# lean-dojo/ReProver

Measured on NVIDIA H100. Metric: premises encoded/sec (reindex_corpus, ByT5-small, seq_len<=512), higher is better.
Workload: dtype bf16

## Files before the change

### reprover_b200/csrc/rpx_encoder.cu

```cuda
#include <math.h>

#include <new>
#include <vector>

#include "rpx_gemm_launch.cuh"
#include "rpx_kernels.cuh"

namespace rpx {

namespace {

constexpr int kBlockN = 128;

int residual_gemm(const void* A, int64_t lda, const void* B, int64_t ldb, int T, int D, int K, float* h32,
                  __nv_bfloat16* h16, float* ss, cudaStream_t st) {
  EpiResidual::Params ep{h32, h16, D, ss, T};
  return launch_gemm<kBlockN, EpiResidual>(A, lda, B, ldb, T, D, K, ep, st);
}

struct LayerW {
  const __nv_bfloat16* qkv;
  const __nv_bfloat16* o;
  const __nv_bfloat16* wi;
  const __nv_bfloat16* wo;
};

struct ProfRec {
  int cls;
  cudaEvent_t a, b;
};

}

}

extern "C" int32_t rpx_t5_relative_bucket(int32_t relative_position, int32_t num_buckets, int32_t max_distance) {
  int nb = num_buckets / 2;
  int ret = relative_position > 0 ? nb : 0;
  int n = relative_position < 0 ? -relative_position : relative_position;
  const int max_exact = nb / 2;
  if (n < max_exact) return ret + n;
  float v = logf((float)n / (float)max_exact) / (float)log((double)max_distance / (double)max_exact) *
            (float)(nb - max_exact);
  int large = max_exact + (int)v;
  if (large > nb - 1) large = nb - 1;
  return ret + large;
}

struct rpx_encoder {
  rpx_t5_config cfg;
  int inner = 0;
  int n_parts = 0;
  int n_parts_lat = 0;
  int latency_tokens = 0;
  size_t layer_bytes = 0;
  const float* emb = nullptr;
  const float* final_ln = nullptr;
  const float* bias_lut = nullptr;
  std::vector<rpx::LayerW> layers;
  float* debug_hidden = nullptr;
  bool profiling = false;
  std::vector<rpx::ProfRec> prof_pending;
  std::vector<cudaEvent_t> event_pool;
  float prof_ms[RPX_N_KERNEL_CLASSES] = {0};
  int64_t prof_launches[RPX_N_KERNEL_CLASSES] = {0};
  std::vector<int32_t> h_cu_tokens;
  std::vector<int32_t> h_lens;
};

namespace rpx {

namespace {

struct PackedLayout {
  size_t emb, final_ln, bias_lut, bucket_tmp, layer0, layer_stride, qkv, o, wi, wo, total;
};

PackedLayout packed_layout(const rpx_t5_config& c) {
  PackedLayout L{};
  const size_t D = c.d_model, inner = (size_t)c.num_heads * c.d_kv, F = c.d_ff;
  size_t off = 0;
  auto take = [&](size_t bytes) {
    size_t o = off;
    off = align_up(off + bytes, 256);
    return o;
  };
  L.emb = take((size_t)c.vocab_size * D * 4);
  L.final_ln = take(D * 4);
  L.bias_lut = take((size_t)c.num_heads * (2 * c.rel_max_distance + 1) * 4);
  L.bucket_tmp = take((size_t)(2 * c.rel_max_distance + 1) * 4);
  L.layer0 = off;
  L.qkv = 0;
  size_t lo = 0;
  auto ltake = [&](size_t bytes) {
    size_t o = lo;
    lo = align_up(lo + bytes, 256);
    return o;
  };
  L.qkv = ltake(3 * inner * D * 2);
  L.o = ltake(D * inner * 2);
  L.wi = ltake(2 * F * D * 2);
// ... 109 lines not shown
  {
    Prof p(e, st, 1);
    EpiStoreBF16::Params ep{ws.qkv, 3 * inner, RowScale{ws.ssA, P, T, inv_d, c.ln_eps}};
    if (T <= kLatSmallMMaxTokens) {
      RPX_TRY((launch_gemm<kLatBlockN, EpiStoreBF16, false, kLatSmallStages, false, kLatSmallM>(ws.h16, D, w.qkv, D, T, 3 * inner,
                                                                                                 D, ep, st, 0, next_weights,
                                                                                                 next_bytes)));
    } else {
      RPX_TRY((launch_gemm<kLatBlockN, EpiStoreBF16, false, kLatStages>(ws.h16, D, w.qkv, D, T, 3 * inner, D, ep, st, 0,
                                                                         next_weights, next_bytes)));
    }
  }
  {
    Prof p(e, st, 2);
    RPX_TRY(launch_t5_attention(ws.qkv, ws.attn, ws.cu_tokens, e->bias_lut, T, S, max_len, c.num_heads, c.d_kv,
                                c.rel_max_distance, st));
  }
  {
    Prof p(e, st, 3);
    EpiResidual::Params ep{ws.h32, ws.h16, D, ws.ssB, T};
    if (T <= kLatSmallMMaxTokens) {
      RPX_TRY((launch_gemm<kLatBlockN, EpiResidualT<true>, false, kLatSmallStages, false, kLatSmallM>(ws.attn, inner, w.o, inner, T,
                                                                                                       D, inner, ep, st)));
    } else {
      RPX_TRY((launch_gemm<kLatBlockN, EpiResidualT<true>, false, kLatStages>(ws.attn, inner, w.o, inner, T, D, inner, ep, st)));
    }
  }
  {
    Prof p(e, st, 4);
    if (T <= kBlockM) {
      EpiGeGLUT<32>::Params ep{ws.ffn, F, RowScale{ws.ssB, P, T, inv_d, c.ln_eps}};
      RPX_TRY((launch_gemm<64, EpiGeGLUT<32>, false, kLatStages, true>(ws.h16, D, w.wi, D, T, 2 * F, D, ep, st)));
    } else {
      EpiGeGLUT<64>::Params ep{ws.ffn, F, RowScale{ws.ssB, P, T, inv_d, c.ln_eps}};
      RPX_TRY((launch_gemm<128, EpiGeGLUT<64>, false, kGemmStages, true>(ws.h16, D, w.wi, D, T, 2 * F, D, ep, st)));
    }
  }
  {
    Prof p(e, st, 5);
    EpiResidual::Params ep{ws.h32, ws.h16, D, ws.ssA, T};
    if (T <= kLatSmallMMaxTokens) {
      RPX_TRY((launch_gemm<kLatBlockN, EpiResidualT<true>, false, kLatSmallStages, false, kLatSmallM>(ws.ffn, F, w.wo, F, T, D, F,
                                                                                                       ep, st)));
    } else {
      RPX_TRY((launch_gemm<kLatBlockN, EpiResidualT<true>, false, kLatStages>(ws.ffn, F, w.wo, F, T, D, F, ep, st)));
    }
  }
  return RPX_OK;
}

int forward(rpx_encoder* e, const Workspace& ws, int T, int S, int max_len, void* d_out, int out_dtype,
            cudaStream_t st) {
  const rpx_t5_config& c = e->cfg;
  const int D = c.d_model, inner = e->inner, F = c.d_ff;
  const bool latency = T <= e->latency_tokens && D % 32 == 0 && (3 * inner) % 32 == 0;
  const int P = latency ? e->n_parts_lat : e->n_parts;
  const float inv_d = 1.0f / (float)D;
  struct PdlScope {
    explicit PdlScope(bool on) { set_pdl_scope(on); }
    ~PdlScope() { set_pdl_scope(false); }
  } pdl_scope(latency || T <= kPdlMaxTokens);
  {
    Prof p(e, st, 0);
    RPX_TRY(launch_embed(ws.ids, e->emb, ws.h32, ws.h16, ws.ssA, T, P, T, D, st));
  }
  auto dump = [&](int slab) -> int {
    if (e->debug_hidden)
      RPX_CUDA_OK(cudaMemcpyAsync(e->debug_hidden + (size_t)slab * T * D, ws.h32, (size_t)T * D * 4,
                                  cudaMemcpyDeviceToDevice, st));
    return RPX_OK;
  };
  RPX_TRY(dump(0));
  for (int l = 0; l < c.num_layers; ++l) {
    const LayerW& w = e->layers[l];
    if (latency) {
      const bool has_next = l + 1 < c.num_layers;
      RPX_TRY(forward_latency_layer(e, ws, w, has_next ? e->layers[l + 1].qkv : nullptr, has_next ? e->layer_bytes : 0, T, S,
                                    max_len, st));
      RPX_TRY(dump(l + 1));
      continue;
    }
    {
      Prof p(e, st, 1);
      EpiStoreBF16::Params ep{ws.qkv, 3 * inner, RowScale{ws.ssA, P, T, inv_d, c.ln_eps}};
      RPX_TRY((launch_gemm<kBlockN, EpiStoreBF16>(ws.h16, D, w.qkv, D, T, 3 * inner, D, ep, st)));
    }
    {
      Prof p(e, st, 2);
      RPX_TRY(launch_t5_attention(ws.qkv, ws.attn, ws.cu_tokens, e->bias_lut, T, S, max_len, c.num_heads, c.d_kv,
                                  c.rel_max_distance, st));
    }
    {
      Prof p(e, st, 3);
      RPX_TRY(residual_gemm(ws.attn, inner, w.o, inner, T, D, inner, ws.h32, ws.h16, ws.ssB, st));
    }
    {
      Prof p(e, st, 4);
      EpiWsGeGLU::Params ep{ws.ffn, F, RowScale{ws.ssB, P, T, inv_d, c.ln_eps}};
      RPX_TRY(launch_gemm_ws<EpiWsGeGLU>(ws.h16, D, w.wi, D, T, 2 * F, D, ep, st));
    }
    {
      Prof p(e, st, 5);
      RPX_TRY(residual_gemm(ws.ffn, F, w.wo, F, T, D, F, ws.h32, ws.h16, ws.ssA, st));
    }
    RPX_TRY(dump(l + 1));
  }
  {
    Prof p(e, st, 6);
    float* scratch = latency && (size_t)F * 2 >= (size_t)D * 4 ? reinterpret_cast<float*>(ws.ffn) : nullptr;
    RPX_TRY(launch_pool_normalize(ws.h32, ws.ssA, T, P, e->final_ln, ws.cu_tokens, d_out, out_dtype, S, D,
                                  c.ln_eps, st, scratch, max_len));
  }
  return RPX_OK;
}

}
}

using namespace rpx;

extern "C" {

size_t rpx_encoder_packed_bytes(const rpx_t5_config* cfg) {
  if (validate_cfg(cfg) != RPX_OK) return 0;
  return packed_layout(*cfg).total;
}

int rpx_encoder_create(const rpx_t5_config* cfg, const rpx_t5_weights* w, void* d_packed, size_t packed_bytes,
                       void* stream, rpx_encoder** out) {
  RPX_TRY(validate_cfg(cfg));
  RPX_REQUIRE(w && d_packed && out, RPX_ERR_INVALID, "rpx_encoder_create: null argument");
  DeviceInfo dev;
  RPX_TRY(get_device_info(&dev));
  const PackedLayout L = packed_layout(*cfg);
  RPX_REQUIRE(packed_bytes >= L.total, RPX_ERR_WORKSPACE, "packed buffer too small: %zu < %zu", packed_bytes, L.total);
  RPX_REQUIRE((reinterpret_cast<uintptr_t>(d_packed) & 255) == 0, RPX_ERR_INVALID, "packed buffer must be 256-byte aligned");
  cudaStream_t st = static_cast<cudaStream_t>(stream);
  uint8_t* base = static_cast<uint8_t*>(d_packed);
  const int D = cfg->d_model, inner = cfg->num_heads * cfg->d_kv, F = cfg->d_ff;

  rpx_encoder* e = new (std::nothrow) rpx_encoder();
  RPX_REQUIRE(e != nullptr, RPX_ERR_INVALID, "out of host memory");
  e->cfg = *cfg;
  e->inner = inner;
  e->n_parts = ceil_div(D, kBlockN) * (EpiResidual::kWarps / 4);
  e->n_parts_lat = ceil_div(D, 32) * (EpiResidual::kWarps / 4);
  auto fail = [&](int code) {
    delete e;
    return code;
  };
#define TRY_E(expr)                        \
  do {                                     \
    int _s = (expr);                       \
    if (_s != RPX_OK) return fail(_s);     \
  } while (0)
#define CUDA_E(expr)                                                                                   \
  do {                                                                                                 \
    cudaError_t _c = (expr);                                                                           \
    if (_c != cudaSuccess) {                                                                           \
      set_error("%s:%d: %s failed: %s", __FILE__, __LINE__, #expr, cudaGetErrorString(_c));           \
      return fail(RPX_ERR_CUDA);                                                                       \
    }                                                                                                  \
  } while (0)

  CUDA_E(cudaMemcpyAsync(base + L.emb, w->d_shared, (size_t)cfg->vocab_size * D * 4, cudaMemcpyDeviceToDevice, st));
  CUDA_E(cudaMemcpyAsync(base + L.final_ln, w->d_final_ln, (size_t)D * 4, cudaMemcpyDeviceToDevice, st));
  e->emb = reinterpret_cast<const float*>(base + L.emb);
  e->final_ln = reinterpret_cast<const float*>(base + L.final_ln);

  const int R = cfg->rel_max_distance, width = 2 * R + 1;
  std::vector<int32_t> buckets(width);
  for (int j = 0; j < width; ++j) buckets[j] = rpx_t5_relative_bucket(j - R, cfg->rel_buckets, R);
  CUDA_E(cudaMemcpyAsync(base + L.bucket_tmp, buckets.data(), (size_t)width * 4, cudaMemcpyHostToDevice, st));
  bias_lut_kernel<<<ceil_div(cfg->num_heads * width, 256), 256, 0, st>>>(
      w->d_rel_bias, reinterpret_cast<const int32_t*>(base + L.bucket_tmp), reinterpret_cast<float*>(base + L.bias_lut),
      cfg->num_heads, width);
  CUDA_E(cudaGetLastError());
  e->bias_lut = reinterpret_cast<const float*>(base + L.bias_lut);

  e->layers.resize(cfg->num_layers);
  for (int l = 0; l < cfg->num_layers; ++l) {
    uint8_t* lb = base + L.layer0 + L.layer_stride * l;
    __nv_bfloat16* qkv = reinterpret_cast<__nv_bfloat16*>(lb + L.qkv);
    __nv_bfloat16* o = reinterpret_cast<__nv_bfloat16*>(lb + L.o);
    __nv_bfloat16* wi = reinterpret_cast<__nv_bfloat16*>(lb + L.wi);
    __nv_bfloat16* wo = reinterpret_cast<__nv_bfloat16*>(lb + L.wo);
    TRY_E(launch_pack_weight(w->h_q[l], w->h_ln0[l], qkv, inner, D, 0, inner, inner, st));
    TRY_E(launch_pack_weight(w->h_k[l], w->h_ln0[l], qkv, inner, D, inner, inner, inner, st));
    TRY_E(launch_pack_weight(w->h_v[l], w->h_ln0[l], qkv, inner, D, 2 * inner, inner, inner, st));
    TRY_E(launch_pack_weight(w->h_o[l], nullptr, o, D, inner, 0, D, D, st));
    TRY_E(launch_pack_weight(w->h_wi0[l], w->h_ln1[l], wi, F, D, 0, 128, 256, st));
    TRY_E(launch_pack_weight(w->h_wi1[l], w->h_ln1[l], wi, F, D, 128, 128, 256, st));
    TRY_E(launch_pack_weight(w->h_wo[l], nullptr, wo, D, F, 0, D, D, st));
    e->layers[l] = LayerW{qkv, o, wi, wo};
    e->layer_bytes = L.layer_stride;
  }
  CUDA_E(cudaStreamSynchronize(st));
#undef TRY_E
#undef CUDA_E
  *out = e;
  return RPX_OK;
}

int rpx_encoder_destroy(rpx_encoder* enc) {
  if (!enc) return RPX_OK;
  for (auto& r : enc->prof_pending) {
    cudaEventDestroy(r.a);
    cudaEventDestroy(r.b);
  }
  for (auto ev : enc->event_pool) cudaEventDestroy(ev);
  delete enc;
  return RPX_OK;
}

size_t rpx_encoder_workspace_bytes(const rpx_encoder* enc, int64_t max_tokens, int64_t max_seqs) {
  if (!enc || max_tokens <= 0 || max_seqs <= 0) return 0;
  return carve(enc, nullptr, max_tokens, max_seqs).total;
}

int rpx_encode_bytes(rpx_encoder* enc, const uint8_t* d_bytes, const int64_t* h_offsets, int32_t n_seqs,
                     int32_t max_seq_len, void* d_out, int32_t out_dtype, void* d_workspace,
                     size_t workspace_bytes, void* stream) {
  RPX_REQUIRE(enc && h_offsets && d_out && d_workspace, RPX_ERR_INVALID, "rpx_encode_bytes: null argument");
  RPX_REQUIRE(n_seqs > 0, RPX_ERR_INVALID, "rpx_encode_bytes: n_seqs=%d", n_seqs);
  RPX_REQUIRE(max_seq_len >= 1, RPX_ERR_INVALID, "rpx_encode_bytes: max_seq_len=%d", max_seq_len);
  RPX_REQUIRE(h_offsets[0] >= 0, RPX_ERR_INVALID, "rpx_encode_bytes: negative offset");
  cudaStream_t st = static_cast<cudaStream_t>(stream);
  auto& cu = enc->h_cu_tokens;
// ... 108 lines not shown
```

### reprover_b200/csrc/rpx_gemm_api.cu

```cuda
#include "rpx_gemm_launch.cuh"

extern "C" int rpx_gemm_bf16_f32(const void* d_A, const void* d_B, float* d_C, int32_t M, int32_t N,
                                 int32_t K, void* stream) {
  using namespace rpx;
  RPX_REQUIRE(d_A && d_B && d_C, RPX_ERR_INVALID, "rpx_gemm_bf16_f32: null pointer");
  EpiWsStoreF32::Params ep{d_C, N};
  return launch_gemm_ws<EpiWsStoreF32>(d_A, K, d_B, K, M, N, K, ep, static_cast<cudaStream_t>(stream));
}

extern "C" int rpx_gemm2_bf16_f32(const void* d_A, const void* d_B, float* d_C, int32_t M, int32_t N, int32_t K,
                                  void* stream) {
  using namespace rpx;
  RPX_REQUIRE(d_A && d_B && d_C, RPX_ERR_INVALID, "rpx_gemm2_bf16_f32: null pointer");
  EpiStoreF32::Params ep{d_C, N};
  return launch_gemm_pair<EpiStoreF32>(d_A, K, d_B, K, M, N, K, ep, static_cast<cudaStream_t>(stream));
}
```

### reprover_b200/csrc/rpx_gemm_launch.cuh

```cuda
#pragma once
#include "rpx_common.cuh"
#include "rpx_gemm.cuh"
#include "rpx_gemm_ws.cuh"

namespace rpx {

constexpr int kGemmStages = 4;

template <int BLOCK_N, class Epi, bool M_FASTEST = false, int STAGES = kGemmStages, bool SPLIT_B = false, int BM = kBlockM>
int launch_gemm(const void* A, int64_t lda, const void* B, int64_t ldb, int M, int N, int K,
                const typename Epi::Params& ep, cudaStream_t stream, int grid_limit = 0, const void* prefetch_ptr = nullptr,
                size_t prefetch_bytes = 0) {
  using Cfg = GemmCfg<BLOCK_N, STAGES, BM>;
  static_assert(BM == kBlockM || (!M_FASTEST && Epi::kWarps == 4), "64-row tiles: encoder epilogues with one warp per lane group");
  RPX_REQUIRE(M > 0 && N > 0 && K > 0, RPX_ERR_INVALID, "gemm: empty problem M=%d N=%d K=%d", M, N, K);
  RPX_REQUIRE(K % kBlockK == 0, RPX_ERR_UNSUPPORTED, "gemm: K=%d must be a multiple of %d", K, kBlockK);
  RPX_REQUIRE(M_FASTEST || N % 32 == 0, RPX_ERR_UNSUPPORTED, "gemm: N=%d must be a multiple of 32", N);
  DeviceInfo dev;
  RPX_TRY(get_device_info(&dev));
  CUtensorMap tmA, tmB;
  RPX_TRY(make_tmap_bf16_2d(&tmA, A, (uint64_t)M, (uint64_t)K, (uint64_t)lda, BM));
  RPX_TRY(make_tmap_bf16_2d(&tmB, B, (uint64_t)N, (uint64_t)K, (uint64_t)ldb, SPLIT_B ? BLOCK_N / 2 : BLOCK_N));
  RPX_REQUIRE(!SPLIT_B || N % BLOCK_N == 0, RPX_ERR_UNSUPPORTED, "gemm: split-B tiles need N %% %d == 0", BLOCK_N);
  const int tiles_m = ceil_div(M, BM);
  const int tiles_n = ceil_div(N, BLOCK_N);
  const size_t smem = Cfg::smem_bytes(Epi::kSmemBytes);
  RPX_REQUIRE(smem <= dev.smem_optin, RPX_ERR_UNSUPPORTED, "gemm: needs %zu B smem, device allows %zu",
              smem, dev.smem_optin);
  auto kern = gemm_tc_kernel<BLOCK_N, STAGES, Epi, M_FASTEST, SPLIT_B, BM>;
  static thread_local int configured_dev = -1;
  if (configured_dev != dev.device) {
    RPX_CUDA_OK(cudaFuncSetAttribute(kern, cudaFuncAttributeMaxDynamicSharedMemorySize, (int)smem));
    configured_dev = dev.device;
  }
  int grid = tiles_m * tiles_n;
  int cap = grid_limit > 0 ? grid_limit : dev.num_sms;
  if (grid > cap) grid = cap;
  L2Prefetch pf{prefetch_ptr, (uint32_t)prefetch_bytes, grid, next_timeline_slot()};
  if (prefetch_ptr != nullptr && prefetch_bytes > 0 && prefetch_bytes < ((size_t)1 << 32) && grid < dev.num_sms)
    grid = dev.num_sms;
  RPX_CUDA_OK(launch_pdl(kern, dim3(grid), dim3(gemm_threads<Epi>()), smem, stream, pdl_enabled(), tmA, tmB, M, N, K, tiles_m,
                         tiles_n, 1, ep, pf));
  return RPX_OK;
}

template <class Epi>
int launch_gemm_ws(const void* A, int64_t lda, const void* B, int64_t ldb, int M, int N, int K,
                   const typename Epi::Params& ep, cudaStream_t stream) {
  RPX_REQUIRE(M > 0 && N > 0 && K > 0, RPX_ERR_INVALID, "gemm: empty problem M=%d N=%d K=%d", M, N, K);
  RPX_REQUIRE(K % kBlockK == 0, RPX_ERR_UNSUPPORTED, "gemm: K=%d must be a multiple of %d", K, kBlockK);
  RPX_REQUIRE(N % 32 == 0, RPX_ERR_UNSUPPORTED, "gemm: N=%d must be a multiple of 32", N);
  DeviceInfo dev;
  RPX_TRY(get_device_info(&dev));
  CUtensorMap tmA, tmB;
  RPX_TRY(make_tmap_bf16_2d(&tmA, A, (uint64_t)M, (uint64_t)K, (uint64_t)lda, kBlockM));
  RPX_TRY(make_tmap_bf16_2d(&tmB, B, (uint64_t)N, (uint64_t)K, (uint64_t)ldb, kWsBlockN));
  const int tiles_m = ceil_div(M, kBlockM);
  const int tiles_n = ceil_div(N, kWsBlockN);
  const size_t smem = WsCfg::kSmemBytes;
  RPX_REQUIRE(smem <= dev.smem_optin, RPX_ERR_UNSUPPORTED, "gemm: needs %zu B smem, device allows %zu", smem,
              dev.smem_optin);
  auto kern = gemm_ws_kernel<Epi>;
  static thread_local int configured_dev = -1;
  if (configured_dev != dev.device) {
    RPX_CUDA_OK(cudaFuncSetAttribute(kern, cudaFuncAttributeMaxDynamicSharedMemorySize, (int)smem));
    configured_dev = dev.device;
  }
  int grid = tiles_m * tiles_n;
  if (grid > dev.num_sms) grid = dev.num_sms;
  RPX_CUDA_OK(launch_pdl(kern, dim3(grid), dim3(kWsThreads), smem, stream, pdl_enabled(), tmA, tmB, M, N, K, tiles_m,
                         tiles_n, ep));
  return RPX_OK;
}

template <class Epi, int STAGES = kGemmStages>
int launch_gemm_pair(const void* A, int64_t lda, const void* B, int64_t ldb, int M, int N, int K,
                     const typename Epi::Params& ep, cudaStream_t stream) {
  constexpr int BLOCK_N = 128;
  using Cfg = GemmCfg<BLOCK_N, STAGES, kBlockM>;
  RPX_REQUIRE(M > 0 && N > 0 && K > 0, RPX_ERR_INVALID, "gemm: empty problem M=%d N=%d K=%d", M, N, K);
  RPX_REQUIRE(K % kBlockK == 0, RPX_ERR_UNSUPPORTED, "gemm: K=%d must be a multiple of %d", K, kBlockK);
  RPX_REQUIRE(N % 32 == 0, RPX_ERR_UNSUPPORTED, "gemm: N=%d must be a multiple of 32", N);
  DeviceInfo dev;
  RPX_TRY(get_device_info(&dev));
  CUtensorMap tmA, tmB;
  RPX_TRY(make_tmap_bf16_2d(&tmA, A, (uint64_t)M, (uint64_t)K, (uint64_t)lda, kBlockM));
  RPX_TRY(make_tmap_bf16_2d(&tmB, B, (uint64_t)N, (uint64_t)K, (uint64_t)ldb, BLOCK_N / 2));
  const int tiles_m = ceil_div(M, kBlockM);
  const int tiles_n = ceil_div(N, BLOCK_N);
  const size_t smem = Cfg::smem_bytes(Epi::kSmemBytes);
  RPX_REQUIRE(smem <= dev.smem_optin, RPX_ERR_UNSUPPORTED, "gemm: needs %zu B smem, device allows %zu", smem,
              dev.smem_optin);
  auto kern = gemm_tc_kernel<BLOCK_N, STAGES, Epi, false, false, kBlockM, true>;
  static thread_local int configured_dev = -1;
  if (configured_dev != dev.device) {
    RPX_CUDA_OK(cudaFuncSetAttribute(kern, cudaFuncAttributeMaxDynamicSharedMemorySize, (int)smem));
    configured_dev = dev.device;
  }
  int pairs = ceil_div(tiles_m, 2) * tiles_n;
  if (pairs > dev.num_sms / 2) pairs = dev.num_sms / 2;
  cudaLaunchConfig_t cfg{};
  cfg.gridDim = dim3(2 * pairs);
  cfg.blockDim = dim3(gemm_threads<Epi>());
  cfg.dynamicSmemBytes = smem;
  cfg.stream = stream;
  cudaLaunchAttribute at[1];
  at[0].id = cudaLaunchAttributeClusterDimension;
  at[0].val.clusterDim.x = 2;
  at[0].val.clusterDim.y = 1;
  at[0].val.clusterDim.z = 1;
  cfg.attrs = at;
  cfg.numAttrs = 1;
  RPX_CUDA_OK(cudaLaunchKernelEx(&cfg, kern, tmA, tmB, M, N, K, tiles_m, tiles_n, 1, ep,
                                 L2Prefetch{nullptr, 0u, 2 * pairs, next_timeline_slot()}));
  return RPX_OK;
}

}
```

### reprover_b200/csrc/rpx_gemm_ws.cuh

```cuda
#pragma once
#include "rpx_gemm.cuh"

namespace rpx {

constexpr int kWsBlockN = 256;
constexpr int kWsStages = 4;
constexpr int kWsThreads = 384;

struct WsCfg {
  static constexpr int kABytes = kBlockM * kBlockK * 2;
  static constexpr int kBBytes = kWsBlockN * kBlockK * 2;
  static constexpr int kStageBytes = kABytes + kBBytes;
  static constexpr size_t kSmemBytes = (size_t)kWsStages * kStageBytes + 1024 + 256;
};

struct FragCtx {
  int m0, n0;
  int n_blk;
  int n_cols;
  int M, N;
  int r0;
  int q;
};

template <class Epi>
__global__ void __launch_bounds__(kWsThreads, 1)
gemm_ws_kernel(const __grid_constant__ CUtensorMap tmA, const __grid_constant__ CUtensorMap tmB, int M, int N, int K,
               int tiles_m, int tiles_n, typename Epi::Params ep) {
  extern __shared__ uint8_t smem_raw[];
  const uint32_t raw_addr = smem_u32(smem_raw);
  uint8_t* smem = smem_raw + ((1024 - (raw_addr & 1023)) & 1023);
  uint8_t* sA = smem;
  uint8_t* sB = smem + kWsStages * WsCfg::kABytes;
  uint64_t* full = reinterpret_cast<uint64_t*>(smem + kWsStages * WsCfg::kStageBytes);
  uint64_t* empty = full + kWsStages;

  const int warp = threadIdx.x >> 5;
  const int wg = warp >> 2;
  const int num_kb = K / kBlockK;
  const int num_tiles = tiles_m * tiles_n;

  if (threadIdx.x == 0) {
    tma_prefetch_desc(&tmA);
    tma_prefetch_desc(&tmB);
    for (int s = 0; s < kWsStages; ++s) {
      mbar_init(&full[s], 1);
      mbar_init(&empty[s], 2 * 128);
    }
    fence_mbar_init();
  }
  __syncthreads();
  pdl_launch_dependents();
  pdl_wait();

  if (wg == 0) {
    setmaxnreg_dec<40>();
    if (warp == 0 && elect_one()) {
      int stage = 0;
      uint32_t phase = 0;
      for (int t = blockIdx.x; t < num_tiles; t += gridDim.x) {
        const int m_blk = t / tiles_n, n_blk = t % tiles_n;
        for (int kb = 0; kb < num_kb; ++kb) {
          mbar_wait(&empty[stage], phase ^ 1);
          mbar_arrive_expect_tx(&full[stage], WsCfg::kStageBytes);
          tma_load_2d(sA + stage * WsCfg::kABytes, &tmA, &full[stage], kb * kBlockK, m_blk * kBlockM);
          tma_load_2d(sB + stage * WsCfg::kBBytes, &tmB, &full[stage], kb * kBlockK, n_blk * kWsBlockN);
          if (++stage == kWsStages) {
            stage = 0;
            phase ^= 1;
          }
        }
      }
    }
  } else {
    setmaxnreg_inc<232>();
    const int cw = wg - 1;
    const int lane = threadIdx.x & 31;
    Epi epi(ep);
    float acc[128];
    int stage = 0;
    uint32_t phase = 0;
    for (int t = blockIdx.x; t < num_tiles; t += gridDim.x) {
      FragCtx c;
      c.n_blk = t % tiles_n;
      c.m0 = (t / tiles_n) * kBlockM;
      c.n0 = c.n_blk * kWsBlockN;
      c.n_cols = N - c.n0 < kWsBlockN ? N - c.n0 : kWsBlockN;
      c.M = M;
      c.N = N;
      c.r0 = c.m0 + 64 * cw + 16 * (warp & 3) + (lane >> 2);
      c.q = lane & 3;
      int prev = 0;
      for (int kb = 0; kb < num_kb; ++kb) {
        mbar_wait(&full[stage], phase);
        const uint64_t a_desc = make_smem_desc_kmajor_sw128(smem_u32(sA + stage * WsCfg::kABytes)) + 512 * cw;
        const uint64_t b_desc = make_smem_desc_kmajor_sw128(smem_u32(sB + stage * WsCfg::kBBytes));
        wgmma_fence_operand(acc);
        wgmma_fence();
#pragma unroll
        for (int k = 0; k < kBlockK / kMmaK; ++k) wgmma_m64n256k16_ss(acc, a_desc + 2 * k, b_desc + 2 * k, (kb | k) != 0);
        wgmma_commit();
        if (kb == 0) epi.prefetch(c);
        if (kb > 0) {
          wgmma_wait<1>();
          mbar_arrive(&empty[prev]);
        }
        prev = stage;
        if (++stage == kWsStages) {
          stage = 0;
          phase ^= 1;
        }
      }
      wgmma_wait<0>();
      wgmma_fence_operand(acc);
      mbar_arrive(&empty[prev]);
      epi.tile(c, acc);
    }
  }
}


struct EpiWsStoreF32 {
  using Params = EpiStoreF32::Params;
  Params p;
  __device__ explicit EpiWsStoreF32(const Params& p_) : p(p_) {}
  __device__ void prefetch(const FragCtx&) {}
  __device__ void tile(const FragCtx& c, const float (&acc)[128]) {
#pragma unroll
    for (int j = 0; j < 32; ++j) {
      if (8 * j < c.n_cols) {
        float* dst = p.C + (size_t)c.r0 * p.ldc + c.n0 + 8 * j + 2 * c.q;
        if (c.r0 < c.M) *reinterpret_cast<float2*>(dst) = make_float2(acc[4 * j], acc[4 * j + 1]);
        if (c.r0 + 8 < c.M) *reinterpret_cast<float2*>(dst + 8 * (size_t)p.ldc) = make_float2(acc[4 * j + 2], acc[4 * j + 3]);
      }
    }
  }
};

struct EpiWsGeGLU {
  struct Params {
    __nv_bfloat16* out;
    int ldo;
    RowScale rs;
  };
  Params p;
  float rs0 = 0.f, rs1 = 0.f;
  __device__ explicit EpiWsGeGLU(const Params& p_) : p(p_) {}
  __device__ void prefetch(const FragCtx& c) {
    rs0 = c.r0 < c.M ? p.rs.get(c.r0) : 0.f;
    rs1 = c.r0 + 8 < c.M ? p.rs.get(c.r0 + 8) : 0.f;
  }
  __device__ void tile(const FragCtx& c, const float (&acc)[128]) {
    __nv_bfloat16* dst = p.out + (size_t)c.r0 * p.ldo + c.n_blk * (kWsBlockN / 2) + 2 * c.q;
#pragma unroll
    for (int j = 0; j < 16; ++j) {
      const float* g = acc + 4 * j;
      const float* u = acc + 4 * (j + 16);
      if (c.r0 < c.M)
        *reinterpret_cast<uint32_t*>(dst + 8 * j) =
            pack_bf16x2(gelu_new(g[0] * rs0) * (u[0] * rs0), gelu_new(g[1] * rs0) * (u[1] * rs0));
      if (c.r0 + 8 < c.M)
        *reinterpret_cast<uint32_t*>(dst + 8 * (size_t)p.ldo + 8 * j) =
            pack_bf16x2(gelu_new(g[2] * rs1) * (u[2] * rs1), gelu_new(g[3] * rs1) * (u[3] * rs1));
    }
  }
};

}
```

### reprover_b200/csrc/rpx_ptx.cuh

```cuda
#pragma once
#include <cuda_runtime.h>
#include <cuda_bf16.h>
#include <stdint.h>

namespace rpx {

#define RPX_DEVICE __device__ __forceinline__

RPX_DEVICE uint32_t smem_u32(const void* p) {
  return static_cast<uint32_t>(__cvta_generic_to_shared(p));
}

RPX_DEVICE uint32_t lane_id() { return threadIdx.x & 31; }

RPX_DEVICE uint32_t elect_one() {
  uint32_t pred = 0;
  asm volatile(
      "{\n"
      ".reg .b32 rx;\n"
      ".reg .pred px;\n"
      "elect.sync rx|px, 0xFFFFFFFF;\n"
      "@px mov.s32 %0, 1;\n"
      "}\n"
      : "+r"(pred));
// ... 123 lines not shown
      "{\n"
      ".reg .b32 ra;\n"
      "mapa.shared::cluster.u32 ra, %0, %1;\n"
      "mbarrier.arrive.release.cluster.shared::cluster.b64 _, [ra];\n"
      "}\n" ::"r"(smem_u32(bar)),
      "r"(cta)
      : "memory");
}

RPX_DEVICE void wgmma_fence() { asm volatile("wgmma.fence.sync.aligned;" ::: "memory"); }
RPX_DEVICE void wgmma_commit() { asm volatile("wgmma.commit_group.sync.aligned;" ::: "memory"); }
template <int N>
RPX_DEVICE void wgmma_wait() {
  asm volatile("wgmma.wait_group.sync.aligned %0;" ::"n"(N) : "memory");
}
template <int R>
RPX_DEVICE void wgmma_fence_operand(float (&d)[R]) {
#pragma unroll
  for (int i = 0; i < R; ++i) asm volatile("" : "+f"(d[i])::"memory");
}

RPX_DEVICE void wgmma_m64n64k16_ss(float (&d)[32], uint64_t desc_a, uint64_t desc_b, uint32_t accumulate) {
  asm volatile(
      "{\n"
      ".reg .pred p;\n"
      "setp.ne.b32 p, %34, 0;\n"
      "wgmma.mma_async.sync.aligned.m64n64k16.f32.bf16.bf16 "
      "{%0, %1, %2, %3, %4, %5, %6, %7, %8, %9, %10, %11, %12, %13, %14, %15, %16, %17, %18, %19, %20, %21, %22, %23, %24, %25, %26, %27, %28, %29, %30, %31}, %32, %33, p, 1, 1, 0, 0;\n"
      "}\n"
      : "+f"(d[0]), "+f"(d[1]), "+f"(d[2]), "+f"(d[3]), "+f"(d[4]), "+f"(d[5]), "+f"(d[6]), "+f"(d[7]), "+f"(d[8]), "+f"(d[9]), "+f"(d[10]), "+f"(d[11]), "+f"(d[12]), "+f"(d[13]), "+f"(d[14]), "+f"(d[15]), "+f"(d[16]), "+f"(d[17]), "+f"(d[18]), "+f"(d[19]), "+f"(d[20]), "+f"(d[21]), "+f"(d[22]), "+f"(d[23]), "+f"(d[24]), "+f"(d[25]), "+f"(d[26]), "+f"(d[27]), "+f"(d[28]), "+f"(d[29]), "+f"(d[30]), "+f"(d[31])
      : "l"(desc_a), "l"(desc_b), "r"(accumulate));
}

RPX_DEVICE void wgmma_m64n128k16_ss(float (&d)[64], uint64_t desc_a, uint64_t desc_b, uint32_t accumulate) {
  asm volatile(
      "{\n"
      ".reg .pred p;\n"
      "setp.ne.b32 p, %66, 0;\n"
      "wgmma.mma_async.sync.aligned.m64n128k16.f32.bf16.bf16 "
      "{%0, %1, %2, %3, %4, %5, %6, %7, %8, %9, %10, %11, %12, %13, %14, %15, %16, %17, %18, %19, %20, %21, %22, %23, %24, %25, %26, %27, %28, %29, %30, %31, %32, %33, %34, %35, %36, %37, %38, %39, %40, %41, %42, %43, %44, %45, %46, %47, %48, %49, %50, %51, %52, %53, %54, %55, %56, %57, %58, %59, %60, %61, %62, %63}, %64, %65, p, 1, 1, 0, 0;\n"
      "}\n"
      : "+f"(d[0]), "+f"(d[1]), "+f"(d[2]), "+f"(d[3]), "+f"(d[4]), "+f"(d[5]), "+f"(d[6]), "+f"(d[7]), "+f"(d[8]), "+f"(d[9]), "+f"(d[10]), "+f"(d[11]), "+f"(d[12]), "+f"(d[13]), "+f"(d[14]), "+f"(d[15]), "+f"(d[16]), "+f"(d[17]), "+f"(d[18]), "+f"(d[19]), "+f"(d[20]), "+f"(d[21]), "+f"(d[22]), "+f"(d[23]), "+f"(d[24]), "+f"(d[25]), "+f"(d[26]), "+f"(d[27]), "+f"(d[28]), "+f"(d[29]), "+f"(d[30]), "+f"(d[31]), "+f"(d[32]), "+f"(d[33]), "+f"(d[34]), "+f"(d[35]), "+f"(d[36]), "+f"(d[37]), "+f"(d[38]), "+f"(d[39]), "+f"(d[40]), "+f"(d[41]), "+f"(d[42]), "+f"(d[43]), "+f"(d[44]), "+f"(d[45]), "+f"(d[46]), "+f"(d[47]), "+f"(d[48]), "+f"(d[49]), "+f"(d[50]), "+f"(d[51]), "+f"(d[52]), "+f"(d[53]), "+f"(d[54]), "+f"(d[55]), "+f"(d[56]), "+f"(d[57]), "+f"(d[58]), "+f"(d[59]), "+f"(d[60]), "+f"(d[61]), "+f"(d[62]), "+f"(d[63])
      : "l"(desc_a), "l"(desc_b), "r"(accumulate));
}

RPX_DEVICE void wgmma_m64n256k16_ss(float (&d)[128], uint64_t desc_a, uint64_t desc_b, uint32_t accumulate) {
  asm volatile(
      "{\n"
      ".reg .pred p;\n"
      "setp.ne.b32 p, %130, 0;\n"
      "wgmma.mma_async.sync.aligned.m64n256k16.f32.bf16.bf16 "
      "{%0, %1, %2, %3, %4, %5, %6, %7, %8, %9, %10, %11, %12, %13, %14, %15, %16, %17, %18, %19, %20, %21, %22, %23, %24, %25, %26, %27, %28, %29, %30, %31, %32, %33, %34, %35, %36, %37, %38, %39, %40, %41, %42, %43, %44, %45, %46, %47, %48, %49, %50, %51, %52, %53, %54, %55, %56, %57, %58, %59, %60, %61, %62, %63, %64, %65, %66, %67, %68, %69, %70, %71, %72, %73, %74, %75, %76, %77, %78, %79, %80, %81, %82, %83, %84, %85, %86, %87, %88, %89, %90, %91, %92, %93, %94, %95, %96, %97, %98, %99, %100, %101, %102, %103, %104, %105, %106, %107, %108, %109, %110, %111, %112, %113, %114, %115, %116, %117, %118, %119, %120, %121, %122, %123, %124, %125, %126, %127}, %128, %129, p, 1, 1, 0, 0;\n"
      "}\n"
      : "+f"(d[0]), "+f"(d[1]), "+f"(d[2]), "+f"(d[3]), "+f"(d[4]), "+f"(d[5]), "+f"(d[6]), "+f"(d[7]), "+f"(d[8]), "+f"(d[9]), "+f"(d[10]), "+f"(d[11]), "+f"(d[12]), "+f"(d[13]), "+f"(d[14]), "+f"(d[15]), "+f"(d[16]), "+f"(d[17]), "+f"(d[18]), "+f"(d[19]), "+f"(d[20]), "+f"(d[21]), "+f"(d[22]), "+f"(d[23]), "+f"(d[24]), "+f"(d[25]), "+f"(d[26]), "+f"(d[27]), "+f"(d[28]), "+f"(d[29]), "+f"(d[30]), "+f"(d[31]), "+f"(d[32]), "+f"(d[33]), "+f"(d[34]), "+f"(d[35]), "+f"(d[36]), "+f"(d[37]), "+f"(d[38]), "+f"(d[39]), "+f"(d[40]), "+f"(d[41]), "+f"(d[42]), "+f"(d[43]), "+f"(d[44]), "+f"(d[45]), "+f"(d[46]), "+f"(d[47]), "+f"(d[48]), "+f"(d[49]), "+f"(d[50]), "+f"(d[51]), "+f"(d[52]), "+f"(d[53]), "+f"(d[54]), "+f"(d[55]), "+f"(d[56]), "+f"(d[57]), "+f"(d[58]), "+f"(d[59]), "+f"(d[60]), "+f"(d[61]), "+f"(d[62]), "+f"(d[63]), "+f"(d[64]), "+f"(d[65]), "+f"(d[66]), "+f"(d[67]), "+f"(d[68]), "+f"(d[69]), "+f"(d[70]), "+f"(d[71]), "+f"(d[72]), "+f"(d[73]), "+f"(d[74]), "+f"(d[75]), "+f"(d[76]), "+f"(d[77]), "+f"(d[78]), "+f"(d[79]), "+f"(d[80]), "+f"(d[81]), "+f"(d[82]), "+f"(d[83]), "+f"(d[84]), "+f"(d[85]), "+f"(d[86]), "+f"(d[87]), "+f"(d[88]), "+f"(d[89]), "+f"(d[90]), "+f"(d[91]), "+f"(d[92]), "+f"(d[93]), "+f"(d[94]), "+f"(d[95]), "+f"(d[96]), "+f"(d[97]), "+f"(d[98]), "+f"(d[99]), "+f"(d[100]), "+f"(d[101]), "+f"(d[102]), "+f"(d[103]), "+f"(d[104]), "+f"(d[105]), "+f"(d[106]), "+f"(d[107]), "+f"(d[108]), "+f"(d[109]), "+f"(d[110]), "+f"(d[111]), "+f"(d[112]), "+f"(d[113]), "+f"(d[114]), "+f"(d[115]), "+f"(d[116]), "+f"(d[117]), "+f"(d[118]), "+f"(d[119]), "+f"(d[120]), "+f"(d[121]), "+f"(d[122]), "+f"(d[123]), "+f"(d[124]), "+f"(d[125]), "+f"(d[126]), "+f"(d[127])
      : "l"(desc_a), "l"(desc_b), "r"(accumulate));
}

RPX_DEVICE void wgmma_m64n64k16_rs_bmn(float (&d)[32], const uint32_t (&a)[4], uint64_t desc_b, uint32_t accumulate) {
  asm volatile(
      "{\n"
      ".reg .pred p;\n"
      "setp.ne.b32 p, %37, 0;\n"
      "wgmma.mma_async.sync.aligned.m64n64k16.f32.bf16.bf16 "
      "{%0, %1, %2, %3, %4, %5, %6, %7, %8, %9, %10, %11, %12, %13, %14, %15, %16, %17, %18, %19, %20, %21, %22, %23, %24, %25, %26, %27, %28, %29, %30, %31}, {%32, %33, %34, %35}, %36, p, 1, 1, 1;\n"
      "}\n"
      : "+f"(d[0]), "+f"(d[1]), "+f"(d[2]), "+f"(d[3]), "+f"(d[4]), "+f"(d[5]), "+f"(d[6]), "+f"(d[7]), "+f"(d[8]), "+f"(d[9]), "+f"(d[10]), "+f"(d[11]), "+f"(d[12]), "+f"(d[13]), "+f"(d[14]), "+f"(d[15]), "+f"(d[16]), "+f"(d[17]), "+f"(d[18]), "+f"(d[19]), "+f"(d[20]), "+f"(d[21]), "+f"(d[22]), "+f"(d[23]), "+f"(d[24]), "+f"(d[25]), "+f"(d[26]), "+f"(d[27]), "+f"(d[28]), "+f"(d[29]), "+f"(d[30]), "+f"(d[31])
      : "r"(a[0]), "r"(a[1]), "r"(a[2]), "r"(a[3]), "l"(desc_b), "r"(accumulate));
}

RPX_DEVICE uint64_t make_smem_desc_sw128(uint32_t smem_addr, uint32_t lbo_bytes) {
  uint64_t d = 0;
  d |= static_cast<uint64_t>((smem_addr & 0x3FFFF) >> 4);
  d |= static_cast<uint64_t>(lbo_bytes >> 4) << 16;
  d |= static_cast<uint64_t>(1024 >> 4) << 32;
  d |= static_cast<uint64_t>(1) << 62;
  return d;
}
RPX_DEVICE uint64_t make_smem_desc_kmajor_sw128(uint32_t smem_addr) { return make_smem_desc_sw128(smem_addr, 16); }
RPX_DEVICE uint64_t make_smem_desc_mnmajor_sw128(uint32_t smem_addr) { return make_smem_desc_sw128(smem_addr, 1024); }

RPX_DEVICE void pdl_wait() { asm volatile("griddepcontrol.wait;" ::: "memory"); }
RPX_DEVICE void pdl_launch_dependents() { asm volatile("griddepcontrol.launch_dependents;" ::: "memory"); }

template <uint32_t N>
RPX_DEVICE void setmaxnreg_dec() { asm volatile("setmaxnreg.dec.sync.aligned.u32 %0;" ::"n"(N)); }
template <uint32_t N>
RPX_DEVICE void setmaxnreg_inc() { asm volatile("setmaxnreg.inc.sync.aligned.u32 %0;" ::"n"(N)); }

RPX_DEVICE uint32_t pack_bf16x2(float lo, float hi) {
  __nv_bfloat162 v = __floats2bfloat162_rn(lo, hi);
  return *reinterpret_cast<uint32_t*>(&v);
}

}
```

Baseline: 4108.

## Add ping-pong warp-specialized GEMM and use it for QKV and out-projection

Templates the warp-specialized GEMM on tile width and adds a 128-wide ping-pong mode. In this mode the two consumer warpgroups take alternating tiles, ordered by named barriers, so one group's epilogue overlaps the other's MMAs. New ping-pong epilogues are added for the QKV projection (bf16 store with RMSNorm row scale from prefetched partial sums) and the attention output projection (residual add plus per-tile sum-of-squares). The cost is more complex barrier and ring-phase bookkeeping, extra register pressure from prefetched partials, and a changed n_parts layout.

```diff
diff --git a/reprover_b200/csrc/rpx_encoder.cu b/reprover_b200/csrc/rpx_encoder.cu
--- a/reprover_b200/csrc/rpx_encoder.cu
+++ b/reprover_b200/csrc/rpx_encoder.cu
@@ -17,6 +17,7 @@
   EpiResidual::Params ep{h32, h16, D, ss, T};
   return launch_gemm<kBlockN, EpiResidual>(A, lda, B, ldb, T, D, K, ep, st);
 }
+static_assert(EpiResidual::kWarps == 4 && EpiWsResidual::kBlockN == kBlockN, "one RMSNorm partial per 128-column tile");
 
 struct LayerW {
   const __nv_bfloat16* qkv;
@@ -292,8 +293,8 @@
     }
     {
       Prof p(e, st, 1);
-      EpiStoreBF16::Params ep{ws.qkv, 3 * inner, RowScale{ws.ssA, P, T, inv_d, c.ln_eps}};
-      RPX_TRY((launch_gemm<kBlockN, EpiStoreBF16>(ws.h16, D, w.qkv, D, T, 3 * inner, D, ep, st)));
+      EpiWsStoreBF16::Params ep{ws.qkv, 3 * inner, RowScale{ws.ssA, P, T, inv_d, c.ln_eps}};
+      RPX_TRY(launch_gemm_ws<EpiWsStoreBF16>(ws.h16, D, w.qkv, D, T, 3 * inner, D, ep, st));
     }
     {
       Prof p(e, st, 2);
@@ -302,7 +303,8 @@
     }
     {
       Prof p(e, st, 3);
-      RPX_TRY(residual_gemm(ws.attn, inner, w.o, inner, T, D, inner, ws.h32, ws.h16, ws.ssB, st));
+      EpiWsResidual::Params ep{ws.h32, ws.h16, D, ws.ssB, T};
+      RPX_TRY(launch_gemm_ws<EpiWsResidual>(ws.attn, inner, w.o, inner, T, D, inner, ep, st));
     }
     {
       Prof p(e, st, 4);
@@ -353,7 +355,7 @@
   RPX_REQUIRE(e != nullptr, RPX_ERR_INVALID, "out of host memory");
   e->cfg = *cfg;
   e->inner = inner;
-  e->n_parts = ceil_div(D, kBlockN) * (EpiResidual::kWarps / 4);
+  e->n_parts = ceil_div(D, kBlockN);
   e->n_parts_lat = ceil_div(D, 32) * (EpiResidual::kWarps / 4);
   auto fail = [&](int code) {
     delete e;
diff --git a/reprover_b200/csrc/rpx_gemm_api.cu b/reprover_b200/csrc/rpx_gemm_api.cu
--- a/reprover_b200/csrc/rpx_gemm_api.cu
+++ b/reprover_b200/csrc/rpx_gemm_api.cu
@@ -4,8 +4,8 @@
                                  int32_t K, void* stream) {
   using namespace rpx;
   RPX_REQUIRE(d_A && d_B && d_C, RPX_ERR_INVALID, "rpx_gemm_bf16_f32: null pointer");
-  EpiWsStoreF32::Params ep{d_C, N};
-  return launch_gemm_ws<EpiWsStoreF32>(d_A, K, d_B, K, M, N, K, ep, static_cast<cudaStream_t>(stream));
+  EpiWsStoreF32<128>::Params ep{d_C, N};
+  return launch_gemm_ws<EpiWsStoreF32<128>>(d_A, K, d_B, K, M, N, K, ep, static_cast<cudaStream_t>(stream));
 }
 
 extern "C" int rpx_gemm2_bf16_f32(const void* d_A, const void* d_B, float* d_C, int32_t M, int32_t N, int32_t K,
diff --git a/reprover_b200/csrc/rpx_gemm_launch.cuh b/reprover_b200/csrc/rpx_gemm_launch.cuh
--- a/reprover_b200/csrc/rpx_gemm_launch.cuh
+++ b/reprover_b200/csrc/rpx_gemm_launch.cuh
@@ -47,6 +47,7 @@
 template <class Epi>
 int launch_gemm_ws(const void* A, int64_t lda, const void* B, int64_t ldb, int M, int N, int K,
                    const typename Epi::Params& ep, cudaStream_t stream) {
+  constexpr int BN = Epi::kBlockN;
   RPX_REQUIRE(M > 0 && N > 0 && K > 0, RPX_ERR_INVALID, "gemm: empty problem M=%d N=%d K=%d", M, N, K);
   RPX_REQUIRE(K % kBlockK == 0, RPX_ERR_UNSUPPORTED, "gemm: K=%d must be a multiple of %d", K, kBlockK);
   RPX_REQUIRE(N % 32 == 0, RPX_ERR_UNSUPPORTED, "gemm: N=%d must be a multiple of 32", N);
@@ -54,10 +55,10 @@
   RPX_TRY(get_device_info(&dev));
   CUtensorMap tmA, tmB;
   RPX_TRY(make_tmap_bf16_2d(&tmA, A, (uint64_t)M, (uint64_t)K, (uint64_t)lda, kBlockM));
-  RPX_TRY(make_tmap_bf16_2d(&tmB, B, (uint64_t)N, (uint64_t)K, (uint64_t)ldb, kWsBlockN));
+  RPX_TRY(make_tmap_bf16_2d(&tmB, B, (uint64_t)N, (uint64_t)K, (uint64_t)ldb, BN));
   const int tiles_m = ceil_div(M, kBlockM);
-  const int tiles_n = ceil_div(N, kWsBlockN);
-  const size_t smem = WsCfg::kSmemBytes;
+  const int tiles_n = ceil_div(N, BN);
+  const size_t smem = WsCfg<BN>::smem_bytes(Epi::kStages);
   RPX_REQUIRE(smem <= dev.smem_optin, RPX_ERR_UNSUPPORTED, "gemm: needs %zu B smem, device allows %zu", smem,
               dev.smem_optin);
   auto kern = gemm_ws_kernel<Epi>;
diff --git a/reprover_b200/csrc/rpx_gemm_ws.cuh b/reprover_b200/csrc/rpx_gemm_ws.cuh
--- a/reprover_b200/csrc/rpx_gemm_ws.cuh
+++ b/reprover_b200/csrc/rpx_gemm_ws.cuh
@@ -3,15 +3,19 @@
 
 namespace rpx {
 
-constexpr int kWsBlockN = 256;
-constexpr int kWsStages = 4;
 constexpr int kWsThreads = 384;
 
+template <int BN>
 struct WsCfg {
+  static_assert(BN == 128 || BN == 256, "ping-pong (128) or cooperative (256) tiles");
+  static constexpr bool kPingPong = BN == 128;
   static constexpr int kABytes = kBlockM * kBlockK * 2;
-  static constexpr int kBBytes = kWsBlockN * kBlockK * 2;
+  static constexpr int kBBytes = BN * kBlockK * 2;
   static constexpr int kStageBytes = kABytes + kBBytes;
-  static constexpr size_t kSmemBytes = (size_t)kWsStages * kStageBytes + 1024 + 256;
+  static constexpr size_t smem_bytes(int stages) { return (size_t)stages * kStageBytes + 1024 + 256; }
+  static constexpr int kH = 256 / BN;
+  static constexpr int kJ = BN / 8;
+  static constexpr __device__ int idx(int h, int e, int j) { return 4 * kJ * h + 4 * j + 2 * e; }
 };
 
 struct FragCtx {
@@ -23,17 +27,33 @@
   int q;
 };
 
+constexpr uint32_t kOrderBar = 1;
+
+RPX_DEVICE void ring_advance(int& stage, uint32_t& phase, int n, int stages) {
+  stage += n % stages;
+  phase ^= (uint32_t)(n / stages) & 1u;
+  if (stage >= stages) {
+    stage -= stages;
+    phase ^= 1u;
+  }
+}
+
 template <class Epi>
 __global__ void __launch_bounds__(kWsThreads, 1)
 gemm_ws_kernel(const __grid_constant__ CUtensorMap tmA, const __grid_constant__ CUtensorMap tmB, int M, int N, int K,
                int tiles_m, int tiles_n, typename Epi::Params ep) {
+  constexpr int BN = Epi::kBlockN;
+  using Cfg = WsCfg<BN>;
+  constexpr bool kPing = Cfg::kPingPong;
+  constexpr int S = Epi::kStages;
+  static_assert(S >= 2 && S <= 14, "barrier block holds at most 14 stages");
   extern __shared__ uint8_t smem_raw[];
   const uint32_t raw_addr = smem_u32(smem_raw);
   uint8_t* smem = smem_raw + ((1024 - (raw_addr & 1023)) & 1023);
   uint8_t* sA = smem;
-  uint8_t* sB = smem + kWsStages * WsCfg::kABytes;
-  uint64_t* full = reinterpret_cast<uint64_t*>(smem + kWsStages * WsCfg::kStageBytes);
-  uint64_t* empty = full + kWsStages;
+  uint8_t* sB = smem + S * Cfg::kABytes;
+  uint64_t* full = reinterpret_cast<uint64_t*>(smem + S * Cfg::kStageBytes);
+  uint64_t* empty = full + S;
 
   const int warp = threadIdx.x >> 5;
   const int wg = warp >> 2;
@@ -43,9 +63,9 @@
   if (threadIdx.x == 0) {
     tma_prefetch_desc(&tmA);
     tma_prefetch_desc(&tmB);
-    for (int s = 0; s < kWsStages; ++s) {
+    for (int s = 0; s < S; ++s) {
       mbar_init(&full[s], 1);
-      mbar_init(&empty[s], 2 * 128);
+      mbar_init(&empty[s], kPing ? 128 : 2 * 128);
     }
     fence_mbar_init();
   }
@@ -62,10 +82,10 @@
         const int m_blk = t / tiles_n, n_blk = t % tiles_n;
         for (int kb = 0; kb < num_kb; ++kb) {
           mbar_wait(&empty[stage], phase ^ 1);
-          mbar_arrive_expect_tx(&full[stage], WsCfg::kStageBytes);
-          tma_load_2d(sA + stage * WsCfg::kABytes, &tmA, &full[stage], kb * kBlockK, m_blk * kBlockM);
-          tma_load_2d(sB + stage * WsCfg::kBBytes, &tmB, &full[stage], kb * kBlockK, n_blk * kWsBlockN);
-          if (++stage == kWsStages) {
+          mbar_arrive_expect_tx(&full[stage], Cfg::kStageBytes);
+          tma_load_2d(sA + stage * Cfg::kABytes, &tmA, &full[stage], kb * kBlockK, m_blk * kBlockM);
+          tma_load_2d(sB + stage * Cfg::kBBytes, &tmB, &full[stage], kb * kBlockK, n_blk * BN);
+          if (++stage == S) {
             stage = 0;
             phase ^= 1;
           }
@@ -80,25 +100,41 @@
     float acc[128];
     int stage = 0;
     uint32_t phase = 0;
-    for (int t = blockIdx.x; t < num_tiles; t += gridDim.x) {
+    const int t_step = kPing ? 2 * (int)gridDim.x : (int)gridDim.x;
+    int t = blockIdx.x;
+    if (kPing && cw == 1) {
+      t += gridDim.x;
+      ring_advance(stage, phase, num_kb, S);
+      named_bar_arrive(kOrderBar, 256);
+    }
+    for (; t < num_tiles; t += t_step) {
       FragCtx c;
       c.n_blk = t % tiles_n;
       c.m0 = (t / tiles_n) * kBlockM;
-      c.n0 = c.n_blk * kWsBlockN;
-      c.n_cols = N - c.n0 < kWsBlockN ? N - c.n0 : kWsBlockN;
+      c.n0 = c.n_blk * BN;
+      c.n_cols = N - c.n0 < BN ? N - c.n0 : BN;
       c.M = M;
       c.N = N;
-      c.r0 = c.m0 + 64 * cw + 16 * (warp & 3) + (lane >> 2);
+      c.r0 = c.m0 + (kPing ? 0 : 64 * cw) + 16 * (warp & 3) + (lane >> 2);
       c.q = lane & 3;
+      if (kPing) named_bar_sync(kOrderBar + cw, 256);
       int prev = 0;
       for (int kb = 0; kb < num_kb; ++kb) {
         mbar_wait(&full[stage], phase);
-        const uint64_t a_desc = make_smem_desc_kmajor_sw128(smem_u32(sA + stage * WsCfg::kABytes)) + 512 * cw;
-        const uint64_t b_desc = make_smem_desc_kmajor_sw128(smem_u32(sB + stage * WsCfg::kBBytes));
+        const uint64_t a_desc = make_smem_desc_kmajor_sw128(smem_u32(sA + stage * Cfg::kABytes));
+        const uint64_t b_desc = make_smem_desc_kmajor_sw128(smem_u32(sB + stage * Cfg::kBBytes));
         wgmma_fence_operand(acc);
         wgmma_fence();
 #pragma unroll
-        for (int k = 0; k < kBlockK / kMmaK; ++k) wgmma_m64n256k16_ss(acc, a_desc + 2 * k, b_desc + 2 * k, (kb | k) != 0);
+        for (int k = 0; k < kBlockK / kMmaK; ++k) {
+          if constexpr (kPing) {
+            wgmma_m64n128k16_ss(*reinterpret_cast<float(*)[64]>(&acc[0]), a_desc + 2 * k, b_desc + 2 * k, (kb | k) != 0);
+            wgmma_m64n128k16_ss(*reinterpret_cast<float(*)[64]>(&acc[64]), a_desc + 512 + 2 * k, b_desc + 2 * k,
+                                (kb | k) != 0);
+          } else {
+            wgmma_m64n256k16_ss(acc, a_desc + 512 * cw + 2 * k, b_desc + 2 * k, (kb | k) != 0);
+          }
+        }
         wgmma_commit();
         if (kb == 0) epi.prefetch(c);
         if (kb > 0) {
@@ -106,43 +142,153 @@
           mbar_arrive(&empty[prev]);
         }
         prev = stage;
-        if (++stage == kWsStages) {
+        if (++stage == S) {
           stage = 0;
           phase ^= 1;
         }
       }
+      if (kPing && t + (int)gridDim.x < num_tiles) named_bar_arrive(kOrderBar + (cw ^ 1), 256);
       wgmma_wait<0>();
       wgmma_fence_operand(acc);
       mbar_arrive(&empty[prev]);
       epi.tile(c, acc);
+      if (kPing) ring_advance(stage, phase, num_kb, S);
     }
   }
 }
 
 
+template <int BN>
 struct EpiWsStoreF32 {
+  static constexpr int kBlockN = BN;
+  static constexpr int kStages = BN == 128 ? 6 : 4;
+  using Cfg = WsCfg<BN>;
   using Params = EpiStoreF32::Params;
   Params p;
   __device__ explicit EpiWsStoreF32(const Params& p_) : p(p_) {}
   __device__ void prefetch(const FragCtx&) {}
   __device__ void tile(const FragCtx& c, const float (&acc)[128]) {
 #pragma unroll
-    for (int j = 0; j < 32; ++j) {
-      if (8 * j < c.n_cols) {
-        float* dst = p.C + (size_t)c.r0 * p.ldc + c.n0 + 8 * j + 2 * c.q;
-        if (c.r0 < c.M) *reinterpret_cast<float2*>(dst) = make_float2(acc[4 * j], acc[4 * j + 1]);
-        if (c.r0 + 8 < c.M) *reinterpret_cast<float2*>(dst + 8 * (size_t)p.ldc) = make_float2(acc[4 * j + 2], acc[4 * j + 3]);
+    for (int h = 0; h < Cfg::kH; ++h)
+#pragma unroll
+      for (int e = 0; e < 2; ++e) {
+        const int m = c.r0 + 64 * h + 8 * e;
+        if (m >= c.M) continue;
+        float* dst = p.C + (size_t)m * p.ldc + c.n0 + 2 * c.q;
+#pragma unroll
+        for (int j = 0; j < Cfg::kJ; ++j) {
+          const int i = Cfg::idx(h, e, j);
+          if (8 * j < c.n_cols) *reinterpret_cast<float2*>(dst + 8 * j) = make_float2(acc[i], acc[i + 1]);
+        }
+      }
+  }
+};
+
+struct EpiWsStoreBF16 {
+  static constexpr int kBlockN = 128;
+  static constexpr int kStages = 4;
+  using Cfg = WsCfg<kBlockN>;
+  using Params = EpiStoreBF16::Params;
+  static constexpr int kRows = 2 * Cfg::kH;
+  static constexpr int kMaxParts = 12;
+  Params p;
+  float v[kRows][kMaxParts];
+  __device__ explicit EpiWsStoreBF16(const Params& p_) : p(p_) {}
+  __device__ static int row(const FragCtx& c, int r) { return c.r0 + 64 * (r >> 1) + 8 * (r & 1); }
+  __device__ void prefetch(const FragCtx& c) {
+    if (p.rs.ss_parts == nullptr || p.rs.n_parts > kMaxParts) return;
+#pragma unroll
+    for (int r = 0; r < kRows; ++r) {
+      const int m = row(c, r);
+#pragma unroll
+      for (int j = 0; j < kMaxParts; ++j)
+        v[r][j] = m < c.M && j < p.rs.n_parts ? p.rs.ss_parts[(size_t)j * p.rs.part_stride + m] : 0.f;
+    }
+  }
+  __device__ float scale(const FragCtx& c, int r) const {
+    if (p.rs.ss_parts == nullptr || p.rs.n_parts > kMaxParts) return p.rs.get(row(c, r));
+    float s = 0.f;
+#pragma unroll
+    for (int j = 0; j < kMaxParts; ++j)
+      if (j < p.rs.n_parts) s += v[r][j];
+    return rsqrtf(s * p.rs.inv_dim + p.rs.eps);
+  }
+  __device__ void tile(const FragCtx& c, const float (&acc)[128]) {
+#pragma unroll
+    for (int r = 0; r < kRows; ++r) {
+      const int h = r >> 1, e = r & 1;
+      const int m = row(c, r);
+      if (m >= c.M) continue;
+      const float rs = scale(c, r);
+      __nv_bfloat16* dst = p.C + (size_t)m * p.ldc + c.n0 + 2 * c.q;
+#pragma unroll
+      for (int j = 0; j < Cfg::kJ; ++j) {
+        const int i = Cfg::idx(h, e, j);
+        if (8 * j < c.n_cols) *reinterpret_cast<uint32_t*>(dst + 8 * j) = pack_bf16x2(acc[i] * rs, acc[i + 1] * rs);
+      }
+    }
+  }
+};
+
+struct EpiWsResidual {
+  static constexpr int kBlockN = 128;
+  static constexpr int kStages = 6;
+  using Cfg = WsCfg<kBlockN>;
+  using Params = EpiResidualParams;
+  Params p;
+  static constexpr int kChunkJ = Cfg::kJ / 2;
+  static constexpr int kChunks = 2 * Cfg::kH * 2;
+  float2 h[kChunkJ];
+  __device__ explicit EpiWsResidual(const Params& p_) : p(p_) {}
+  __device__ static int chunk_row(const FragCtx& c, int k) { return c.r0 + 64 * (k >> 2) + 8 * ((k >> 1) & 1); }
+  __device__ __forceinline__ void load_chunk(const FragCtx& c, int k, float2 (&hh)[kChunkJ]) const {
+    const int m = chunk_row(c, k), j0 = kChunkJ * (k & 1);
+    const float* src = p.h32 + (size_t)m * p.ld + c.n0 + 2 * c.q;
+#pragma unroll
+    for (int j = 0; j < kChunkJ; ++j)
+      hh[j] = m < c.M && 8 * (j0 + j) < c.n_cols ? *reinterpret_cast<const float2*>(src + 8 * (j0 + j))
+                                                  : make_float2(0.f, 0.f);
+  }
+  __device__ void prefetch(const FragCtx& c) { load_chunk(c, 0, h); }
+  __device__ void tile(const FragCtx& c, const float (&acc)[128]) {
+    float ss = 0.f;
+#pragma unroll
+    for (int k = 0; k < kChunks; ++k) {
+      const int hh = k >> 2, e = (k >> 1) & 1, j0 = kChunkJ * (k & 1);
+      const int m = chunk_row(c, k);
+      float2 hn[kChunkJ];
+      if (k + 1 < kChunks) load_chunk(c, k + 1, hn);
+      float* d32 = p.h32 + (size_t)m * p.ld + c.n0 + 2 * c.q;
+      __nv_bfloat16* d16 = p.h16 + (size_t)m * p.ld + c.n0 + 2 * c.q;
+#pragma unroll
+      for (int j = 0; j < kChunkJ; ++j) {
+        const int i = Cfg::idx(hh, e, j0 + j);
+        const float x = h[j].x + acc[i], y = h[j].y + acc[i + 1];
+        ss += x * x + y * y;
+        if (m < c.M && 8 * (j0 + j) < c.n_cols) {
+          *reinterpret_cast<float2*>(d32 + 8 * (j0 + j)) = make_float2(x, y);
+          *reinterpret_cast<uint32_t*>(d16 + 8 * (j0 + j)) = pack_bf16x2(x, y);
+        }
+      }
+      if (k & 1) {
+        ss += __shfl_xor_sync(0xffffffffu, ss, 1);
+        ss += __shfl_xor_sync(0xffffffffu, ss, 2);
+        if (c.q == 0 && m < c.M) p.ss_out[(size_t)c.n_blk * p.ss_stride + m] = ss;
+        ss = 0.f;
+      }
+      if (k + 1 < kChunks) {
+#pragma unroll
+        for (int j = 0; j < kChunkJ; ++j) h[j] = hn[j];
       }
     }
   }
 };
 
 struct EpiWsGeGLU {
-  struct Params {
-    __nv_bfloat16* out;
-    int ldo;
-    RowScale rs;
-  };
+  static constexpr int kBlockN = 256;
+  static constexpr int kStages = 4;
+  using Cfg = WsCfg<kBlockN>;
+  using Params = EpiGeGLUT<64>::Params;
   Params p;
   float rs0 = 0.f, rs1 = 0.f;
   __device__ explicit EpiWsGeGLU(const Params& p_) : p(p_) {}
@@ -151,7 +297,7 @@
     rs1 = c.r0 + 8 < c.M ? p.rs.get(c.r0 + 8) : 0.f;
   }
   __device__ void tile(const FragCtx& c, const float (&acc)[128]) {
-    __nv_bfloat16* dst = p.out + (size_t)c.r0 * p.ldo + c.n_blk * (kWsBlockN / 2) + 2 * c.q;
+    __nv_bfloat16* dst = p.out + (size_t)c.r0 * p.ldo + c.n_blk * (kBlockN / 2) + 2 * c.q;
 #pragma unroll
     for (int j = 0; j < 16; ++j) {
       const float* g = acc + 4 * j;
diff --git a/reprover_b200/csrc/rpx_ptx.cuh b/reprover_b200/csrc/rpx_ptx.cuh
--- a/reprover_b200/csrc/rpx_ptx.cuh
+++ b/reprover_b200/csrc/rpx_ptx.cuh
@@ -229,6 +229,9 @@
 RPX_DEVICE void pdl_wait() { asm volatile("griddepcontrol.wait;" ::: "memory"); }
 RPX_DEVICE void pdl_launch_dependents() { asm volatile("griddepcontrol.launch_dependents;" ::: "memory"); }
 
+RPX_DEVICE void named_bar_sync(uint32_t id, uint32_t n) { asm volatile("bar.sync %0, %1;" ::"r"(id), "r"(n) : "memory"); }
+RPX_DEVICE void named_bar_arrive(uint32_t id, uint32_t n) { asm volatile("bar.arrive %0, %1;" ::"r"(id), "r"(n) : "memory"); }
+
 template <uint32_t N>
 RPX_DEVICE void setmaxnreg_dec() { asm volatile("setmaxnreg.dec.sync.aligned.u32 %0;" ::"n"(N)); }
 template <uint32_t N>
```

After: 4126, median of 6. No clear change (+0.4%).
